# nekStab/nekStab_next

Hardware: AMD Instinct MI355X
Metric: Arnoldi-step GB/s (achieved HBM) + Ritz-value rel-err, N=1e8 m=128 (higher is better)
Workload: dtype f64

## Files before the change

### include/nekkrylov.h

```cpp
#ifndef NEKKRYLOV_H
#define NEKKRYLOV_H

#include <stddef.h>
#include <stdint.h>

#ifdef __cplusplus
extern "C" {
#endif

#define NKV_ABI_VERSION 3

#define NKV_TILE 4096
#define NKV_MAX_COLS 1024
#define NKV_ROT_MAX_OUT 256

#define NKV_OK 0
#define NKV_EINVAL 1
#define NKV_EHIP 2
#define NKV_ENAN 3
#define NKV_ESHAPE 4
#define NKV_ECALLBACK 5
#define NKV_EBREAKDOWN 6

#define NKV_TIME 0x1u
// ... 58 lines not shown
                void* stream);
int nkv_normalize_store(const nkv_layout* L, const double* f, const double* nrm2_dev, double* q_next,
                        double* beta_dev, unsigned flags, void* stream);
int nkv_mgs2_step(const nkv_layout* L, const double* w, const double* Q, int j, double* f, double* q_out,
                  double* hcol_dev, void* ws, unsigned flags, void* stream);
int nkv_axpy_dot(const nkv_layout* L, const double* w, double* f, const double* alpha_dev, const double* qa,
                 const double* qb, double* out_dev, void* ws, unsigned flags, void* stream);

int nkv_block_dot2(const nkv_layout* L, const double* w, const double* Q, int j, const double* x,
                   const double* y, double* h_dev, void* ws, unsigned flags, void* stream);
int nkv_dcgs2_coef(int m, const double* hq_dev, const double* hw_dev, const double* nrm_prev_dev, double* H_dev,
                   int64_t ldh, double* coef_dev, void* ws, void* stream);
int nkv_dcgs2_update(const nkv_layout* L, const double* w, const double* Q, int m, const double* coef_dev,
                     double* qj, const double* win, double* fout, double* nrm2_dev, void* ws, unsigned flags,
                     void* stream);

int nkv_mgs_icwy_solve(int j, double* G, int64_t ldg, const double* grow, const double* b, double* x,
                       void* stream);

int nkv_gkl_coef(int side, int m, const double* hq_dev, const double* hw_dev, double* M_dev, int64_t ldm,
                 double* A_self, double* r_self, const double* A_other, const double* r_other, int64_t lda,
                 double* coef_dev, void* ws, void* stream);

typedef int (*nkv_matvec_fn)(void* user, const double* x, double* y, void* stream);
typedef int (*nkv_allreduce_fn)(void* user, double* buf, int n, void* stream);
size_t nkv_arnoldi_scratch_doubles(int m);
int nkv_arnoldi_dcgs2(const nkv_layout* L, const double* w, double* Q, int mstart, int mend, double* H_dev,
                      int64_t ldh, double* f, double* scratch_dev, void* ws, nkv_matvec_fn matvec, void* mv_user,
                      nkv_allreduce_fn allreduce, void* ar_user, unsigned flags, void* stream);

// ... 22 lines not shown
int nkv_rotate_plan(const nkv_layout* L, int k, int ldv, int n_out, int* path, int* inst, int* wg_threads,
                    int* rows_per_tile);

#define NKV_STREAM_BLOCK_DOT 1
#define NKV_STREAM_BLOCK_UPDATE 2
#define NKV_STREAM_UPDATE_DOT 3
#define NKV_STREAM_BLOCK_DOT2 4
#define NKV_STREAM_DCGS2_UPDATE 5
#define NKV_STREAM_AXPY_DOT 6
#define NKV_STREAM_BLAS1 7
#define NKV_STREAM_OP_DIAG 8
#define NKV_STREAM_FINISH 9
#define NKV_STREAM_SPLIT 10
#define NKV_STREAM_LOOP_TILES 1
#define NKV_STREAM_LOOP_UNITS 2
typedef struct nkv_plan {
    int64_t kernel, pairs, nw, cpw, wg_threads, rows_per_tile, tiles, grid_x, grid_y, launches, band_tiles,
        last_grid_x, work_loop, units, fields_per_block, partial_slots, partial_cols;
} nkv_plan;
int nkv_stream_plan(const nkv_layout* L, int op, int j, unsigned flags, nkv_plan* plan);

int nkv_op_diag(const nkv_layout* L, const double* d, const double* x, double* y, double time_scale,
                void* stream);
int nkv_op_rot2(const nkv_layout* L, const double* c, const double* s, const double* d_rest,
                const double* x, double* y, int transpose, void* stream);
int nkv_op_cdiag(const nkv_layout* L, const double* cr, const double* ci, const double* x, double* y, int conj,
                 void* stream);

int nkv_wavemaker(const nkv_layout* L, const double* dRe, const double* dIm, const double* aRe, const double* aIm,
                  double* out, int ncomp, void* stream);
// ... 130 lines not shown
```

### nekstab_next_amd/_lib.py

```python
from __future__ import annotations

import ctypes
import os
from ctypes import CFUNCTYPE, POINTER, Structure, c_char_p, c_double, c_int, c_int32, c_int64, c_size_t, c_uint, c_uint64, c_void_p

import torch

_HERE = os.path.dirname(os.path.abspath(__file__))
LIB_PATH = os.path.join(_HERE, "libnekkrylov.so")

NKV_ABI_VERSION = 3
NKV_TILE = 4096
NKV_MAX_COLS = 1024
NKV_ROT_MAX_OUT = 256
NKV_GS_MAX_FIELDS = 64
NKV_ROT_PATH_FEW, NKV_ROT_PATH_WIDE, NKV_ROT_PATH_STREAM, NKV_ROT_PATH_CHUNKED = 1, 2, 3, 4
(NKV_STREAM_BLOCK_DOT, NKV_STREAM_BLOCK_UPDATE, NKV_STREAM_UPDATE_DOT, NKV_STREAM_BLOCK_DOT2, NKV_STREAM_DCGS2_UPDATE,
 NKV_STREAM_AXPY_DOT, NKV_STREAM_BLAS1, NKV_STREAM_OP_DIAG, NKV_STREAM_FINISH, NKV_STREAM_SPLIT) = range(1, 11)
NKV_STREAM_LOOP_TILES, NKV_STREAM_LOOP_UNITS = 1, 2
NKV_OK, NKV_EINVAL, NKV_EHIP, NKV_ENAN, NKV_ESHAPE, NKV_ECALLBACK, NKV_EBREAKDOWN = 0, 1, 2, 3, 4, 5, 6
NKV_TIME = 0x1
NKV_ACCUMULATE = 0x2
NKV_OVERWRITE = 0x4
NKV_NORM2 = 0x8
NKV_TIME_DOT = 0x10
NKV_X_IS_LAST = 0x20
NKV_MGS2 = 0x40
NKV_MGS_ICWY = 0x100
NKV_MGS_LAGGED = 0x200
NKV_CHECK_BREAKDOWN = 0x80
NKV_SFD_MONITOR = 0x400
NKV_TDF_STORE = 0x800
NKV_BF_IMAG = 0x1000
NKV_BF_PERTURBATION = 0x2000
# ... 51 lines not shown
    "nkv_copy": (c_int, [_L, _P, _P, c_uint, _P]),
    "nkv_scal": (c_int, [_L, _P, c_double, c_uint, _P]),
    "nkv_axpby": (c_int, [_L, _P, c_double, _P, c_double, c_uint, _P]),
    "nkv_sub3": (c_int, [_L, _P, _P, _P, c_uint, _P]),
    "nkv_axpy_dev": (c_int, [_L, _P, _P, c_double, _P, c_uint, _P]),
    "nkv_normalize_dev": (c_int, [_L, _P, _P, _P, c_uint, _P]),
    "nkv_dot": (c_int, [_L, _P, _P, _P, _P, _P, c_uint, _P]),
    "nkv_block_dot": (c_int, [_L, _P, _P, c_int, _P, _P, _P, c_uint, _P]),
    "nkv_block_update": (c_int, [_L, _P, _P, c_int, _P, _P, _P, _P, c_uint, _P]),
    "nkv_block_update_dot": (c_int, [_L, _P, _P, c_int, _P, _P, _P, _P, c_uint, _P]),
    "nkv_arnoldi_finish": (c_int, [_L, _P, _P, _P, c_int, _P, _P, _P, c_uint, _P]),
    "nkv_block_dot2": (c_int, [_L, _P, _P, c_int, _P, _P, _P, _P, c_uint, _P]),
    "nkv_dcgs2_coef": (c_int, [c_int, _P, _P, _P, _P, c_int64, _P, _P, _P]),
    "nkv_mgs_icwy_solve": (c_int, [c_int, _P, c_int64, _P, _P, _P, _P]),
    "nkv_dcgs2_update": (c_int, [_L, _P, _P, c_int, _P, _P, _P, _P, _P, _P, c_uint, _P]),
    "nkv_arnoldi_scratch_doubles": (c_size_t, [c_int]),
    "nkv_arnoldi_dcgs2": (c_int, [_L, _P, _P, c_int, c_int, _P, c_int64, _P, _P, _P, MATVEC_FN, _P, ALLREDUCE_FN, _P,
                                  c_uint, _P]),
    "nkv_update_hessenberg": (c_int, [_L, _P, _P, c_int, _P, _P, _P, _P, _P, ALLREDUCE_FN, _P, c_uint, _P]),
    "nkv_gmres_dcgs2": (c_int, [_L, _P, _P, c_int, c_double, c_double, _P, c_int64, _P, _P, _P, MATVEC_FN, _P,
                                ALLREDUCE_FN, _P, _P, _P, c_uint, _P]),
    "nkv_arnoldi_factorization": (c_int, [_L, _P, _P, c_int, c_int, _P, c_int64, _P, _P, _P, MATVEC_FN, _P,
                                          ALLREDUCE_FN, _P, c_uint, _P]),
    "nkv_combine": (c_int, [_L, _P, c_int, _P, _P, c_uint, _P]),
    "nkv_normalize_store": (c_int, [_L, _P, _P, _P, _P, c_uint, _P]),
    "nkv_mgs2_step": (c_int, [_L, _P, _P, c_int, _P, _P, _P, _P, c_uint, _P]),
    "nkv_axpy_dot": (c_int, [_L, _P, _P, _P, _P, _P, _P, _P, c_uint, _P]),
    "nkv_rotate": (c_int, [_L, _P, c_int, _P, c_int, _P]),
    "nkv_rotate_cols": (c_int, [_L, _P, c_int, _P, c_int, c_int, _P]),
    "nkv_rotate_plan": (c_int, [_L, c_int, c_int, c_int, POINTER(c_int), POINTER(c_int), POINTER(c_int),
# ... 107 lines not shown
```

### nekstab_next_amd/arnoldi.py

```python
from __future__ import annotations

import numpy as np
import torch

from . import _lib
from ._lib import NKV_NORM2, NKV_TIME, NKV_TIME_DOT, NKV_X_IS_LAST
from .operators import LinearOperator
from .vector import Basis, NekContext, NekVector


class HessenbergDev:

    def __init__(self, ctx: NekContext, k: int):
        self.ctx, self.k = ctx, k
        self.t = torch.zeros((k, k + 1), dtype=torch.float64, device=ctx.device)

    def col_ptr(self, c: int) -> int:
        return self.t[c].data_ptr()

    def download(self) -> np.ndarray:
        return np.asfortranarray(self.t.detach().cpu().numpy().T)

    def upload(self, H: np.ndarray) -> None:
        self.t.copy_(torch.as_tensor(np.ascontiguousarray(np.asarray(H, dtype=np.float64).T)).to(self.ctx.device))
# ... 68 lines not shown
                out = h[i + 1:i + 2] if not last else (h2[0:1] if p == 0 else nrm)
                ctx.call("nkv_axpy_dot", w, f.ptr, h[i:i + 1].data_ptr(), Q.col_ptr(i), qn, out.data_ptr(), ws, fl,
                         st)
                ctx.comm.allreduce_(out)
    else:
        raise ValueError(f"unknown orthogonalisation mode {mode!r}")
    if ctx.timer:
        ctx.timer.begin("finish")
    ctx.call("nkv_arnoldi_finish", f.ptr, nrm.data_ptr(), out_ptr, j, h1.data_ptr(), h2.data_ptr(),
             hcol_ptr, 0, st)
    if ctx.timer:
        ctx.timer.end("finish", 16.0 * ctx.layout.N)


def _dcgs2_step(ctx: NekContext, Q: Basis, Hd: HessenbergDev, j: int, f: NekVector, first: bool,
                nrm2: torch.Tensor | None = None) -> None:
    w, ws, st = ctx.w.data_ptr(), ctx.ws.data_ptr(), ctx.stream
    lay, tm = ctx.layout, ctx.timer
    tf = NKV_TIME if ctx.time_in_dot else 0
    m = j - 1
    h = ctx.hd[: 2 * j]
    hp, cp = h.data_ptr(), ctx.coef.data_ptr()
    u = Q.col_ptr(m)
    if tm:
        tm.begin("block_dot2")
    ctx.call("nkv_block_dot2", w, Q.ptr, j, u, f.ptr, hp, ws, tf | NKV_X_IS_LAST, st)
    if tm:
        tm.end("block_dot2", 8.0 * ((j - 1) * lay.N_w + 2 * lay.N_w + lay.n_v))
    ctx.comm.allreduce_(h)
    nprev = None if first else (nrm2.data_ptr() if nrm2 is not None else hp + 8 * m)
    ctx.call_nl("nkv_dcgs2_coef", m, hp, hp + 8 * j, nprev, Hd.t.data_ptr(), Hd.k + 1, cp, ws, st)
    if tm:
        tm.begin("dcgs2_update")
    ctx.call("nkv_dcgs2_update", w, Q.ptr, m, cp, u, f.ptr, Q.col_ptr(j), None if nrm2 is None else nrm2.data_ptr(),
             ws, NKV_TIME | (NKV_TIME_DOT if tf else 0), st)
    if tm:
        tm.end("dcgs2_update", 8.0 * (m * lay.N + 4 * lay.N) + (0.0 if nrm2 is None else 8.0 * lay.n_v))
    if nrm2 is not None:
        ctx.comm.allreduce_(nrm2)


def _dcgs2_close(ctx: NekContext, Q: Basis, Hd: HessenbergDev, m: int) -> None:
    w, ws, st = ctx.w.data_ptr(), ctx.ws.data_ptr(), ctx.stream
    lay, tm = ctx.layout, ctx.timer
    tf = NKV_TIME if ctx.time_in_dot else 0
    h, coef = ctx.hd[: m + 1], ctx.coef
    u = Q.col_ptr(m)
    if tm:
        tm.begin("block_dot")
    ctx.call("nkv_block_dot", w, Q.ptr, m + 1, u, h.data_ptr(), ws, tf, st)
    if tm:
        tm.end("block_dot", 8.0 * ((m + 1) * lay.N_w + lay.N_w + lay.n_v))
    ctx.comm.allreduce_(h)
    ctx.call_nl("nkv_dcgs2_coef", m, h.data_ptr(), None, h.data_ptr() + 8 * m, Hd.t.data_ptr(), Hd.k + 1,
                coef.data_ptr(), ws, st)
    if tm:
        tm.begin("block_update")
    ctx.call("nkv_block_update", w, Q.ptr, m, h.data_ptr(), u, None, ws, NKV_TIME, st)
    if tm:
        tm.end("block_update", 8.0 * (m * lay.N + 2 * lay.N))
    ctx.call("nkv_normalize_dev", u, coef[2 * m + 3:].data_ptr(), None, 0, st)


def _icwy_gram(ctx: NekContext, Q: Basis, mstart: int) -> torch.Tensor:
    ldg = ctx.max_cols + 1
    G = getattr(ctx, "_icwy_G", None)
    if G is None:
        G = ctx._icwy_G = torch.zeros((ldg, ldg), dtype=torch.float64, device=ctx.device)
    w, ws, st = ctx.w.data_ptr(), ctx.ws.data_ptr(), ctx.stream
    tf = NKV_TIME if ctx.time_in_dot else 0
    for i in range(1, mstart - 1):
        ctx.call("nkv_block_dot", w, Q.ptr, i, Q.col_ptr(i), G[i].data_ptr(), ws, tf, st)
        ctx.comm.allreduce_(G[i, :i])
    return G


# ... 183 lines not shown
        raise ValueError("basis too small")
    if f is None:
        f = ctx.vector()
    if mode == "dcgs2-native":
        if on_step is None:
            if mend > ctx.max_cols or mend + 1 > Hd.k + 1:
                raise ValueError(f"step {mend} exceeds max_cols {ctx.max_cols} / H size {Hd.k}")
            _dcgs2_native(ctx, op, Q, Hd, mstart, mend, f, transpose)
            return
        mode = "dcgs2"
    if mode == "dcgs2" and on_step is not None:
        if mend > ctx.max_cols or mend + 1 > Hd.k + 1:
            raise ValueError(f"step {mend} exceeds max_cols {ctx.max_cols} / H size {Hd.k}")
        for mstep in range(mstart, mend + 1):
            (op.rmatvec if transpose else op.matvec)(Q[mstep - 1], f)
            _dcgs2_step(ctx, Q, Hd, mstep, f, first=(mstep == mstart))
            if mstep > mstart:
                on_step(mstep - 1)
        _dcgs2_close(ctx, Q, Hd, mend)
        on_step(mend)
        return
    if mode == "mgs2-lagged-native":
        if on_step is None:
            if mend > ctx.max_cols or mend + 1 > Hd.k + 1:
                raise ValueError(f"step {mend} exceeds max_cols {ctx.max_cols} / H size {Hd.k}")
            _dcgs2_native(ctx, op, Q, Hd, mstart, mend, f, transpose, entry="nkv_arnoldi_factorization",
                          flags=_lib.NKV_MGS_LAGGED)
            return
        mode = "mgs2-lagged"
    if mode == "mgs2-lagged":
        if mend > ctx.max_cols or mend + 1 > Hd.k + 1:
# ... 17 lines not shown
            _icwy_step(ctx, Q, Hd, mstep, f, G)
            if on_step is not None:
                on_step(mstep)
        return
    if mode in ("cgs2-native", "mgs2-native") and on_step is None:
        if mend > ctx.max_cols or mend + 1 > Hd.k + 1:
            raise ValueError(f"step {mend} exceeds max_cols {ctx.max_cols} / H size {Hd.k}")
        _dcgs2_native(ctx, op, Q, Hd, mstart, mend, f, transpose, entry="nkv_arnoldi_factorization",
                      flags=_lib.NKV_MGS2 if mode == "mgs2-native" else 0)
        return
    if mode == "dcgs2" and on_step is None:
        if mend > ctx.max_cols or mend + 1 > Hd.k + 1:
            raise ValueError(f"step {mend} exceeds max_cols {ctx.max_cols} / H size {Hd.k}")
        for mstep in range(mstart, mend + 1):
            (op.rmatvec if transpose else op.matvec)(Q[mstep - 1], f)
            _dcgs2_step(ctx, Q, Hd, mstep, f, first=(mstep == mstart))
        _dcgs2_close(ctx, Q, Hd, mend)
        return
    if mode == "dcgs2":
        mode = "cgs2"
    for mstep in range(mstart, mend + 1):
        x = Q[mstep - 1]
        (op.rmatvec if transpose else op.matvec)(x, f)
        update_hessenberg_matrix(ctx, Q, mstep, f, Hd, mode)
        if on_step is not None:
            on_step(mstep)


class FactorizationGraph:

    def __init__(self, ctx: NekContext, op: LinearOperator, Q: Basis, Hd: HessenbergDev, f: NekVector,
# ... 26 lines not shown
```

### nekstab_next_amd/csrc/core.hip

```cpp
#include "nkv_internal.h"

namespace nkvi {

thread_local char g_err[512] = "";

int fail(int code, const char* fmt, ...) {
    va_list ap;
    va_start(ap, fmt);
    vsnprintf(g_err, sizeof(g_err), fmt, ap);
    va_end(ap);
    return code;
}

int device_cus() {
    static int cus[64] = {0};
    int dev = 0;
    if (hipGetDevice(&dev) != hipSuccess || dev < 0 || dev >= 64) return 256;
    if (!cus[dev]) {
        int n = 0;
        cus[dev] = (hipDeviceGetAttribute(&n, hipDeviceAttributeMultiprocessorCount, dev) == hipSuccess && n > 0)
                       ? n : 256;
    }
    return cus[dev];
}
// ... 172 lines not shown
            set_tile_grid(&p, L, large ? NKV_DC_PAIRS : NKV_PAIRS_SMALL, NKV_DC_G < kMaxBlocks ? NKV_DC_G : kMaxBlocks);
            if (!(flags & NKV_NORM2)) {
                set_bands(&p, NKV_DC_ROUNDS, true);
                break;
            }
            set_bands(&p, 0, true);
            const int64_t tpf = L->sv / p.rows_per_tile;
            if (!(tpf < p.grid_x && j >= 8)) {
                p.work_loop = NKV_STREAM_LOOP_UNITS;
                p.units = tpf + (p.tiles - tpf * L->n_wf);
            }
            p.partial_slots = p.grid_x;
            p.partial_cols = 1;
            break;
        }
        case NKV_STREAM_AXPY_DOT: {
            set_tile_grid(&p, L, NKV_PAIRS_SMALL, kMaxBlocks);
            set_bands(&p, NKV_AXD_ROUNDS, true);
            p.partial_slots = p.tiles > 0 ? p.grid_x : 0;
            p.partial_cols = 1;
            break;
        }
        case NKV_STREAM_BLAS1:
        case NKV_STREAM_FINISH:
        case NKV_STREAM_OP_DIAG: {
            p.pairs = kStreamUnr;
            p.wg_threads = kThreads;
            p.rows_per_tile = (int64_t)2 * kThreads * kStreamUnr;
            p.tiles = rows / p.rows_per_tile;
            p.grid_x = grid_for(op == NKV_STREAM_BLAS1 ? rows / 2 + 1 : rows / 2);
// ... 28 lines not shown
```

### nekstab_next_amd/csrc/drivers.hip

```cpp
#include "nkv_internal.h"

#include <vector>

extern "C" {

static size_t icwy_scratch_doubles(int m) { return (size_t)(4 * (m + 1) + 2) + (size_t)(m + 1) * (size_t)(m + 1); }
size_t nkv_arnoldi_scratch_doubles(int m) {
    const size_t base = (size_t)(2 * (m + 1) + 4 * m + 16), icwy = icwy_scratch_doubles(m);
    return base > icwy ? base : icwy;
}

static constexpr double kBreakdownTol = 1e-8;

static int check_breakdown(const double* H_dev, int64_t ldh, int c0, int c1, void* ws, void* stream) {
    if (c0 < 0) c0 = 0;
    if (c1 <= c0) return NKV_OK;
    hipStream_t st = S(stream);
    const size_t n = (size_t)ldh * (size_t)(c1 - c0);
    double* h = static_cast<double*>(malloc(n * sizeof(double)));
    if (!h) return fail(NKV_EINVAL, "breakdown check: host allocation of %zu doubles failed", n);
    int flag = 0;
    hipError_t e = hipMemcpyAsync(h, H_dev + (int64_t)c0 * ldh, n * sizeof(double), hipMemcpyDeviceToHost, st);
    if (e == hipSuccess) e = hipMemcpyAsync(&flag, nan_flag_of(ws), sizeof(int), hipMemcpyDeviceToHost, st);
    if (e == hipSuccess) e = hipStreamSynchronize(st);
// ... 34 lines not shown
    if (mend < mstart) return NKV_OK;
    if (ldh < mend + 1) return fail(NKV_EINVAL, "ldh=%lld < mend+1=%d", (long long)ldh, mend + 1);
    const unsigned tf = (flags & NKV_TIME_DOT) ? NKV_TIME : 0u;
    double* hd = scratch_dev;
    double* coef = scratch_dev + 2 * (mend + 1);
    auto col = [L, Q](int c) { return Q + (int64_t)c * L->ld; };
    for (int j = mstart; j <= mend; ++j) {
        const int m = j - 1;
        double* u = col(m);
        int rc = matvec(mv_user, u, f, stream);
        if (rc != 0) return fail(NKV_ECALLBACK, "matvec callback returned %d at step %d", rc, j);
        CHECK(nkv_block_dot2(L, w, Q, j, u, f, hd, ws, tf | NKV_X_IS_LAST, stream));
        if (allreduce && (rc = allreduce(ar_user, hd, 2 * j, stream)) != 0)
            return fail(NKV_ECALLBACK, "allreduce callback returned %d at step %d", rc, j);
        CHECK(nkv_dcgs2_coef(m, hd, hd + j, j == mstart ? nullptr : hd + m, H_dev, ldh, coef, ws, stream));
        CHECK(nkv_dcgs2_update(L, w, Q, m, coef, u, f, col(j), nullptr, ws, NKV_TIME, stream));
    }
    const int m = mend;
    double* u = col(m);
    CHECK(nkv_block_dot(L, w, Q, m + 1, u, hd, ws, tf, stream));
    if (allreduce) {
        const int rc = allreduce(ar_user, hd, m + 1, stream);
        if (rc != 0) return fail(NKV_ECALLBACK, "allreduce callback returned %d (closing step)", rc);
    }
    CHECK(nkv_dcgs2_coef(m, hd, nullptr, hd + m, H_dev, ldh, coef, ws, stream));
    CHECK(nkv_block_update(L, w, Q, m, hd, u, nullptr, ws, NKV_TIME, stream));
    CHECK(nkv_normalize_dev(L, u, coef + 2 * m + 3, nullptr, 0, stream));
    return (flags & NKV_CHECK_BREAKDOWN) ? check_breakdown(H_dev, ldh, mstart - 1, mend, ws, stream) : NKV_OK;
}

int nkv_gmres_dcgs2(const nkv_layout* L, const double* w, double* Q, int kmax, double beta, double tol2,
                    double* H_dev, int64_t ldh, double* f, double* scratch_dev, void* ws, nkv_matvec_fn matvec,
                    void* mv_user, nkv_allreduce_fn allreduce, void* ar_user, double* res_hist, int* k_out,
                    unsigned flags, void* stream) {
    CHECK(check_layout(L));
    CHECK(check_ptr(Q, "Q"));
    CHECK(check_ptr(f, "f"));
    CHECK(check_ptr(w, "w"));
    CHECK(check_ptr(ws, "ws"));
    if (!matvec) return fail(NKV_EINVAL, "matvec callback is NULL");
    if (!H_dev || !scratch_dev || !res_hist || !k_out) return fail(NKV_EINVAL, "H/scratch/res_hist/k_out is NULL");
    if (kmax < 1 || kmax + 1 > NKV_MAX_COLS) return fail(NKV_EINVAL, "kmax=%d outside 1..%d", kmax, NKV_MAX_COLS - 1);
// ... 325 lines not shown
```

### nekstab_next_amd/csrc/gram_schmidt.hip

```cpp
#include "nkv_internal.h"

namespace {

template <bool OVERWRITE, bool NORM, int kPairs>
__global__ __launch_bounds__(kThreads) void k_block_update(const double* __restrict__ Q, int64_t ld,
                                                           int j, const double* __restrict__ h,
                                                           double* __restrict__ f,
                                                           const double* __restrict__ w, int64_t sv,
                                                           int tiles_per_field, int tiles_w,
                                                           int tiles_total, int64_t time_off,
                                                           int do_time,
                                                           double* __restrict__ partials, int t_lo,
                                                           int acc_part) {
    constexpr int kTile = kThreads * kPairs * 2;
    __shared__ double lds4[4];
    if (do_time && blockIdx.x == 0 && threadIdx.x < 64) {
        double s = 0.0;
        for (int c = threadIdx.x; c < j; c += 64) s = fma(Q[time_off + (int64_t)c * ld], h[c], s);
        s = wave_sum(s);
        if (threadIdx.x == 0) f[time_off] = OVERWRITE ? s : f[time_off] - s;
    }
    double nrm = 0.0;
    for (int t = t_lo + blockIdx.x; t < tiles_total; t += gridDim.x) {
        const int64_t r0 = (int64_t)t * kTile + 2 * threadIdx.x;
        double2 acc[kPairs];
#pragma unroll
        for (int k = 0; k < kPairs; ++k) {
            if (OVERWRITE) acc[k] = make_double2(0.0, 0.0);
            else acc[k] = ld2(f + r0 + k * 2 * kThreads);
        }
        const double* qb = Q + r0;
        int c = 0;
        for (; c + 4 <= j; c += 4) {
            double2 q[4][kPairs];
#pragma unroll
// ... 6 lines not shown
#pragma unroll
                for (int k = 0; k < kPairs; ++k) {
                    acc[k].x = fma(hc, q[u][k].x, acc[k].x);
                    acc[k].y = fma(hc, q[u][k].y, acc[k].y);
                }
            }
        }
        for (; c < j; ++c) {
            const double hc = OVERWRITE ? h[c] : -h[c];
#pragma unroll
            for (int k = 0; k < kPairs; ++k) {
                const double2 q = ldq(qb + (int64_t)c * ld + k * 2 * kThreads);
                acc[k].x = fma(hc, q.x, acc[k].x);
                acc[k].y = fma(hc, q.y, acc[k].y);
            }
        }
#pragma unroll
        for (int k = 0; k < kPairs; ++k) st2(f + r0 + k * 2 * kThreads, acc[k]);
        if (NORM && t < tiles_w) {
            const int64_t wr = r0 - (int64_t)(t / tiles_per_field) * sv;
#pragma unroll
            for (int k = 0; k < kPairs; ++k) {
                const double2 wv = ld2(w + wr + k * 2 * kThreads);
                nrm = fma(wv.x * acc[k].x, acc[k].x, nrm);
                nrm = fma(wv.y * acc[k].y, acc[k].y, nrm);
            }
        }
    }
    if (NORM) {
        nrm = block_sum(nrm, lds4);
// ... 480 lines not shown
#pragma unroll
                for (int k = 0; k < kPairs; ++k) {
                    nrm = fma(wv[k].x * af[k].x, af[k].x, nrm);
                    nrm = fma(wv[k].y * af[k].y, af[k].y, nrm);
                }
            }
        } else {
            dcgs2_tile<kPairs>(Q, ld, m, a, x, rinv, yc, sc, qj, win, f,
                               (int64_t)(tiles_w + u - tiles_per_field) * kTile + 2 * threadIdx.x, af);
        }
    }
    nrm = block_sum(nrm, lds4);
    if (threadIdx.x == 0) partials[blockIdx.x] = nrm;
}

template <int P>
int launch_block_update_p(const nkv_layout* L, const nkv_plan& p, const double* w, const double* Q, int j,
                          const double* h_dev, double* f, double* part, unsigned flags, hipStream_t st) {
    const bool over = (flags & NKV_OVERWRITE) != 0;
    const bool norm = (flags & NKV_NORM2) != 0;
    const int tpf = (int)(L->sv / p.rows_per_tile);
    const int tiles_w = tpf * L->n_wf;
    const int tiles_total = (int)p.tiles;
    const int64_t T = rows_of(L);
    const int dt = (flags & NKV_TIME) ? 1 : 0;
    auto kern = over ? (norm ? k_block_update<true, true, P> : k_block_update<true, false, P>)
                     : (norm ? k_block_update<false, true, P> : k_block_update<false, false, P>);
    for (int64_t i = 0; i < p.launches; ++i) {
        const int lo = (int)(i * p.band_tiles);
        const int hi = lo + p.band_tiles < tiles_total ? (int)(lo + p.band_tiles) : tiles_total;
        const int64_t gb = i + 1 == p.launches ? p.last_grid_x : p.grid_x;
        hipLaunchKernelGGL(kern, dim3((unsigned)gb), dim3(kThreads), 0, st, Q, L->ld, j, h_dev, f, w, L->sv, tpf, tiles_w,
                           hi, T, lo == 0 ? dt : 0, part, lo, lo == 0 ? 0 : 1);
        NKV_LAUNCHED();
    }
    return NKV_OK;
}

__global__ __launch_bounds__(kThreads) void k_mgs_icwy_solve(int j, double* __restrict__ G, int64_t ldg,
                                                             const double* __restrict__ grow,
                                                             const double* b, double* x) {
    extern __shared__ double xs[];
    for (int i = threadIdx.x; i < j; i += kThreads) xs[i] = b[i];
    if (grow)
        for (int k = threadIdx.x; k < j - 1; k += kThreads) G[(int64_t)(j - 1) * ldg + k] = grow[k];
    for (int k = 0; k + 1 < j; ++k) {
        __syncthreads();
        const double xk = xs[k];
// ... 23 lines not shown
        CHECK(check_ptr(w, "w"));
        CHECK(check_ptr(ws, "ws"));
        if (!nrm2_dev) return fail(NKV_EINVAL, "nrm2_dev is NULL");
    }
    double* part = ws ? partials_of(ws) : nullptr;
    hipStream_t st = S(stream);
    const int g = (int)p.grid_x;
    const int64_t T = rows_of(L);
    if (p.pairs == NKV_PAIRS) CHECK(launch_block_update_p<NKV_PAIRS>(L, p, w, Q, j, h_dev, f, part, flags, st));
    else CHECK(launch_block_update_p<NKV_PAIRS_SMALL>(L, p, w, Q, j, h_dev, f, part, flags, st));
    if (norm) {
        const bool tdot = (flags & NKV_TIME_DOT) && L->rank0;
        CHECK(launch_reduce_cols(1, part, g, nrm2_dev, tdot ? f + T : nullptr, (int64_t)0, tdot ? f + T : nullptr, nullptr, 1 << 30, nan_flag_of(ws), st));
    }
    return NKV_OK;
}

int nkv_block_update_dot(const nkv_layout* L, const double* w, const double* Q, int j, const double* h_dev,
                         double* f, double* hout_dev, void* ws, unsigned flags, void* stream) {
    CHECK(check_layout(L));
    CHECK(check_ptr(w, "w"));
    CHECK(check_ptr(Q, "Q"));
    CHECK(check_ptr(f, "f"));
    CHECK(check_ptr(ws, "ws"));
    if (!h_dev || !hout_dev) return fail(NKV_EINVAL, "h_dev/hout_dev is NULL");
    nkv_plan p;
    CHECK(nkv_stream_plan(L, NKV_STREAM_UPDATE_DOT, j, flags, &p));
    const unsigned upd_flags = (flags & NKV_TIME) ? NKV_TIME : 0u;
    const unsigned dot_flags = (flags & NKV_TIME_DOT) ? NKV_TIME : 0u;
    if (p.kernel == NKV_STREAM_SPLIT) {
// ... 158 lines not shown
                      : (nrm2_dev ? k_dcgs2_update<NKV_PAIRS_SMALL, true> : k_dcgs2_update<NKV_PAIRS_SMALL, false>);
    for (int64_t i = 0; i < p.launches; ++i) {
        const int lo = (int)(i * p.band_tiles);
        const int hi = lo + p.band_tiles < tiles_total ? (int)(lo + p.band_tiles) : tiles_total;
        const int64_t gb = i + 1 == p.launches ? p.last_grid_x : p.grid_x;
        hipLaunchKernelGGL(kern, dim3((unsigned)gb), dim3(kThreads), 0, st, Q, L->ld, m, coef_dev, qj, win, fout, w, L->sv,
                           tpf, tiles_w, tiles_total, T, lo == 0 ? dt : 0, part, lo, hi);
        NKV_LAUNCHED();
    }
    if (!nrm2_dev) return NKV_OK;
    const bool tdot = (flags & NKV_TIME_DOT) && L->rank0;
    CHECK(launch_reduce_cols(1, part, g, nrm2_dev, tdot ? fout + T : nullptr, (int64_t)0, tdot ? fout + T : nullptr, nullptr, 1 << 30, nan_flag_of(ws), st));
    return NKV_OK;
}

int nkv_combine(const nkv_layout* L, const double* Q, int k, const double* y_dev, double* out, unsigned flags,
                void* stream) {
    return nkv_block_update(L, nullptr, Q, k, y_dev, out, nullptr, nullptr,
                            (flags & ~(unsigned)NKV_NORM2) | NKV_OVERWRITE, stream);
}

}
```

### nekstab_next_amd/csrc/nkv_internal.h

```cpp
#pragma once

#include <hip/hip_runtime.h>

#include <cmath>
#include <cstdarg>
#include <cstdio>
#include <cstdlib>
#include <cstring>

#include "nekkrylov.h"

#ifndef NKV_PAIRS
#define NKV_PAIRS 8
#endif
#ifndef NKV_PAIRS_SMALL
#define NKV_PAIRS_SMALL 4
#endif
#ifndef NKV_SMALL_TILES
#define NKV_SMALL_TILES 2048
#endif
#ifndef NKV_COLU
#define NKV_COLU 4
#endif
#ifndef NKV_NT
// ... 37 lines not shown
#endif
#ifndef NKV_AXD_ROUNDS
#define NKV_AXD_ROUNDS 0
#endif
#ifndef NKV_UPD_SMALL_J
#define NKV_UPD_SMALL_J 2
#endif
#ifndef NKV_FUSE_SMALL_J
#define NKV_FUSE_SMALL_J 12
#endif
static_assert(NKV_FUSE_SMALL_J >= 0 && NKV_FUSE_SMALL_J <= 16,
              "the 4-wave fused pass instantiates at most 16 columns (NKV_FUSE(4, 4))");
#ifndef NKV_FUSE_ROUNDS
#define NKV_FUSE_ROUNDS 0
#endif
#ifndef NKV_DC_ROUNDS
#define NKV_DC_ROUNDS 2
#endif
#ifndef NKV_STREAM_ROUNDS
#define NKV_STREAM_ROUNDS 2
#endif
#ifndef NKV_D2_MAXB
#define NKV_D2_MAXB 256
#endif
#ifndef NKV_D2_SMALL_B
#define NKV_D2_SMALL_B 512
#endif
#ifndef NKV_DOT_SMALL_B
#define NKV_DOT_SMALL_B 512
#endif
// ... 296 lines not shown
```

### nekstab_next_amd/vector.py

```python
from __future__ import annotations

import ctypes

import numpy as np
import torch

from . import _lib
from ._lib import NKV_OVERWRITE, NKV_TIME
from .comm import Comm
from .layout import NekLayout


def _ptr(t: torch.Tensor) -> int:
    return t.data_ptr()


class NekContext:

    def __init__(self, layout: NekLayout, weights=None, comm: Comm | None = None, max_cols: int = 256,
                 device: torch.device | int | None = None, time_in_dot: bool = False):
        if not 1 <= max_cols < _lib.NKV_MAX_COLS:
            raise ValueError(f"max_cols={max_cols} outside 1..{_lib.NKV_MAX_COLS - 1}")
        _lib.require_gpu()
        self.comm = comm if comm is not None else Comm()
# ... 258 lines not shown
                _lib.NKV_ROT_PATH_CHUNKED: "chunked"}


def rotate_plan(layout, k: int, n_out: int, ldv: int | None = None) -> tuple[str, int, int, int]:
    L = layout.c_struct() if isinstance(layout, NekLayout) else layout
    out = [ctypes.c_int(0) for _ in range(4)]
    rc = _lib.load().nkv_rotate_plan(ctypes.byref(L), int(k), int(k if ldv is None else ldv), int(n_out),
                                     *[ctypes.byref(o) for o in out])
    _lib.check(rc, "nkv_rotate_plan")
    return ROTATE_PATHS[out[0].value], out[1].value, out[2].value, out[3].value


STREAM_OPS = {"block_dot": _lib.NKV_STREAM_BLOCK_DOT, "block_update": _lib.NKV_STREAM_BLOCK_UPDATE,
              "update_dot": _lib.NKV_STREAM_UPDATE_DOT, "block_dot2": _lib.NKV_STREAM_BLOCK_DOT2,
              "dcgs2_update": _lib.NKV_STREAM_DCGS2_UPDATE, "axpy_dot": _lib.NKV_STREAM_AXPY_DOT,
              "blas1": _lib.NKV_STREAM_BLAS1, "op_diag": _lib.NKV_STREAM_OP_DIAG, "finish": _lib.NKV_STREAM_FINISH}
_STREAM_KERNELS = {**{v: k for k, v in STREAM_OPS.items()}, _lib.NKV_STREAM_SPLIT: "split"}
_STREAM_LOOPS = {0: None, _lib.NKV_STREAM_LOOP_TILES: "tiles", _lib.NKV_STREAM_LOOP_UNITS: "units"}


class StreamPlan(dict):

    __getattr__ = dict.__getitem__


def stream_plan(layout, op: str, j: int = 1, flags: int = 0) -> StreamPlan:
    L = layout.c_struct() if isinstance(layout, NekLayout) else layout
    p = _lib.nkv_plan()
    _lib.check(_lib.load().nkv_stream_plan(ctypes.byref(L), STREAM_OPS[op], int(j), int(flags), ctypes.byref(p)),
               "nkv_stream_plan")
    out = StreamPlan((name, int(getattr(p, name))) for name, _ in p._fields_)
# ... 12 lines not shown
```

Before: 6764.

## Fuse closing block-dot into final DCGS2 update and scale in block update

The last Arnoldi step now uses a new fused kernel that performs the DCGS2 update and computes the closing dot products against all basis columns while the tiles are still in registers, so the separate block_dot pass over Q is no longer needed. The closing normalize is folded into the block update through a scaled variant that multiplies by the inverse norm before storing. Together these drop one full read of the basis and one vector pass per Arnoldi cycle. The cost is a more complex kernel with LDS cross-wave reductions and a per-tile barrier, plus many template instantiations. Large m or very large row counts fall back to the split path.

Measured after the change: 6753. About the same (-0.2%).

```diff
diff --git a/include/nekkrylov.h b/include/nekkrylov.h
--- a/include/nekkrylov.h
+++ b/include/nekkrylov.h
@@ -96,6 +96,11 @@
 int nkv_dcgs2_update(const nkv_layout* L, const double* w, const double* Q, int m, const double* coef_dev,
                      double* qj, const double* win, double* fout, double* nrm2_dev, void* ws, unsigned flags,
                      void* stream);
+int nkv_dcgs2_update_dot(const nkv_layout* L, const double* w, const double* Q, int m, const double* coef_dev,
+                         double* qj, const double* win, double* fout, double* hout_dev, void* ws, unsigned flags,
+                         void* stream);
+int nkv_block_update_scaled(const nkv_layout* L, const double* Q, int j, const double* h_dev, double* f,
+                            const double* nrm2_dev, void* stream);
 
 int nkv_mgs_icwy_solve(int j, double* G, int64_t ldg, const double* grow, const double* b, double* x,
                        void* stream);
@@ -148,6 +153,7 @@
 #define NKV_STREAM_SPLIT 10
 #define NKV_STREAM_LOOP_TILES 1
 #define NKV_STREAM_LOOP_UNITS 2
+#define NKV_PLAN_DCGS2_UPDATE_DOT 12
 typedef struct nkv_plan {
     int64_t kernel, pairs, nw, cpw, wg_threads, rows_per_tile, tiles, grid_x, grid_y, launches, band_tiles,
         last_grid_x, work_loop, units, fields_per_block, partial_slots, partial_cols;
diff --git a/nekstab_next_amd/_lib.py b/nekstab_next_amd/_lib.py
--- a/nekstab_next_amd/_lib.py
+++ b/nekstab_next_amd/_lib.py
@@ -18,6 +18,7 @@
 (NKV_STREAM_BLOCK_DOT, NKV_STREAM_BLOCK_UPDATE, NKV_STREAM_UPDATE_DOT, NKV_STREAM_BLOCK_DOT2, NKV_STREAM_DCGS2_UPDATE,
  NKV_STREAM_AXPY_DOT, NKV_STREAM_BLAS1, NKV_STREAM_OP_DIAG, NKV_STREAM_FINISH, NKV_STREAM_SPLIT) = range(1, 11)
 NKV_STREAM_LOOP_TILES, NKV_STREAM_LOOP_UNITS = 1, 2
+NKV_PLAN_DCGS2_UPDATE_DOT = 12
 NKV_OK, NKV_EINVAL, NKV_EHIP, NKV_ENAN, NKV_ESHAPE, NKV_ECALLBACK, NKV_EBREAKDOWN = 0, 1, 2, 3, 4, 5, 6
 NKV_TIME = 0x1
 NKV_ACCUMULATE = 0x2
@@ -99,6 +100,8 @@
     "nkv_dcgs2_coef": (c_int, [c_int, _P, _P, _P, _P, c_int64, _P, _P, _P]),
     "nkv_mgs_icwy_solve": (c_int, [c_int, _P, c_int64, _P, _P, _P, _P]),
     "nkv_dcgs2_update": (c_int, [_L, _P, _P, c_int, _P, _P, _P, _P, _P, _P, c_uint, _P]),
+    "nkv_dcgs2_update_dot": (c_int, [_L, _P, _P, c_int, _P, _P, _P, _P, _P, _P, c_uint, _P]),
+    "nkv_block_update_scaled": (c_int, [_L, _P, c_int, _P, _P, _P, _P]),
     "nkv_arnoldi_scratch_doubles": (c_size_t, [c_int]),
     "nkv_arnoldi_dcgs2": (c_int, [_L, _P, _P, c_int, c_int, _P, c_int64, _P, _P, _P, MATVEC_FN, _P, ALLREDUCE_FN, _P,
                                   c_uint, _P]),
diff --git a/nekstab_next_amd/arnoldi.py b/nekstab_next_amd/arnoldi.py
--- a/nekstab_next_amd/arnoldi.py
+++ b/nekstab_next_amd/arnoldi.py
@@ -106,7 +106,9 @@
 
 
 def _dcgs2_step(ctx: NekContext, Q: Basis, Hd: HessenbergDev, j: int, f: NekVector, first: bool,
-                nrm2: torch.Tensor | None = None) -> None:
+                nrm2: torch.Tensor | None = None, last: bool = False) -> None:
+    if last and nrm2 is not None:
+        raise ValueError("last=True: the closing dots supply the norm; nrm2 must be None")
     w, ws, st = ctx.w.data_ptr(), ctx.ws.data_ptr(), ctx.stream
     lay, tm = ctx.layout, ctx.timer
     tf = NKV_TIME if ctx.time_in_dot else 0
@@ -124,6 +126,12 @@
     ctx.call_nl("nkv_dcgs2_coef", m, hp, hp + 8 * j, nprev, Hd.t.data_ptr(), Hd.k + 1, cp, ws, st)
     if tm:
         tm.begin("dcgs2_update")
+    if last:
+        ctx.call("nkv_dcgs2_update_dot", w, Q.ptr, m, cp, u, f.ptr, Q.col_ptr(j), hp, ws,
+                 NKV_TIME | (NKV_TIME_DOT if tf else 0), st)
+        if tm:
+            tm.end("dcgs2_update", 8.0 * (m * lay.N + 4 * lay.N + lay.n_v))
+        return
     ctx.call("nkv_dcgs2_update", w, Q.ptr, m, cp, u, f.ptr, Q.col_ptr(j), None if nrm2 is None else nrm2.data_ptr(),
              ws, NKV_TIME | (NKV_TIME_DOT if tf else 0), st)
     if tm:
@@ -133,25 +141,18 @@
 
 
 def _dcgs2_close(ctx: NekContext, Q: Basis, Hd: HessenbergDev, m: int) -> None:
-    w, ws, st = ctx.w.data_ptr(), ctx.ws.data_ptr(), ctx.stream
+    st = ctx.stream
     lay, tm = ctx.layout, ctx.timer
-    tf = NKV_TIME if ctx.time_in_dot else 0
     h, coef = ctx.hd[: m + 1], ctx.coef
     u = Q.col_ptr(m)
-    if tm:
-        tm.begin("block_dot")
-    ctx.call("nkv_block_dot", w, Q.ptr, m + 1, u, h.data_ptr(), ws, tf, st)
-    if tm:
-        tm.end("block_dot", 8.0 * ((m + 1) * lay.N_w + lay.N_w + lay.n_v))
     ctx.comm.allreduce_(h)
     ctx.call_nl("nkv_dcgs2_coef", m, h.data_ptr(), None, h.data_ptr() + 8 * m, Hd.t.data_ptr(), Hd.k + 1,
-                coef.data_ptr(), ws, st)
+                coef.data_ptr(), ctx.ws.data_ptr(), st)
     if tm:
         tm.begin("block_update")
-    ctx.call("nkv_block_update", w, Q.ptr, m, h.data_ptr(), u, None, ws, NKV_TIME, st)
+    ctx.call("nkv_block_update_scaled", Q.ptr, m, h.data_ptr(), u, coef[2 * m + 3:].data_ptr(), st)
     if tm:
         tm.end("block_update", 8.0 * (m * lay.N + 2 * lay.N))
-    ctx.call("nkv_normalize_dev", u, coef[2 * m + 3:].data_ptr(), None, 0, st)
 
 
 def _icwy_gram(ctx: NekContext, Q: Basis, mstart: int) -> torch.Tensor:
@@ -365,7 +366,7 @@
             raise ValueError(f"step {mend} exceeds max_cols {ctx.max_cols} / H size {Hd.k}")
         for mstep in range(mstart, mend + 1):
             (op.rmatvec if transpose else op.matvec)(Q[mstep - 1], f)
-            _dcgs2_step(ctx, Q, Hd, mstep, f, first=(mstep == mstart))
+            _dcgs2_step(ctx, Q, Hd, mstep, f, first=(mstep == mstart), last=(mstep == mend))
             if mstep > mstart:
                 on_step(mstep - 1)
         _dcgs2_close(ctx, Q, Hd, mend)
@@ -413,7 +414,7 @@
             raise ValueError(f"step {mend} exceeds max_cols {ctx.max_cols} / H size {Hd.k}")
         for mstep in range(mstart, mend + 1):
             (op.rmatvec if transpose else op.matvec)(Q[mstep - 1], f)
-            _dcgs2_step(ctx, Q, Hd, mstep, f, first=(mstep == mstart))
+            _dcgs2_step(ctx, Q, Hd, mstep, f, first=(mstep == mstart), last=(mstep == mend))
         _dcgs2_close(ctx, Q, Hd, mend)
         return
     if mode == "dcgs2":
diff --git a/nekstab_next_amd/csrc/core.hip b/nekstab_next_amd/csrc/core.hip
--- a/nekstab_next_amd/csrc/core.hip
+++ b/nekstab_next_amd/csrc/core.hip
@@ -210,6 +210,29 @@
             p.partial_cols = 1;
             break;
         }
+        case NKV_PLAN_DCGS2_UPDATE_DOT: {
+            if (j < 0 || j + 2 > NKV_MAX_COLS) return fail(NKV_EINVAL, "m=%d outside 0..%d", j, NKV_MAX_COLS - 2);
+            if (j > NKV_DCF_MAX_M || rows >= (int64_t)1 << 29) {
+                p.kernel = NKV_STREAM_SPLIT;
+                break;
+            }
+            p.nw = j <= NKV_FUSE_SMALL_J ? 4 : 8;
+            p.cpw = j > 0 ? (j + p.nw - 1) / p.nw : 1;
+            p.pairs = 1;
+            p.wg_threads = p.nw * 64;
+            p.rows_per_tile = kFuseRows;
+            p.tiles = rows / kFuseRows;
+            p.grid_x = p.tiles < NKV_DCF_G ? p.tiles : NKV_DCF_G;
+            if (p.grid_x < 1) p.grid_x = 1;
+            p.grid_y = 1;
+            p.work_loop = NKV_STREAM_LOOP_TILES;
+            p.units = p.tiles;
+            p.fields_per_block = 1;
+            set_bands(&p, 0, true);
+            p.partial_slots = p.grid_x;
+            p.partial_cols = j + 2;
+            break;
+        }
         case NKV_STREAM_AXPY_DOT: {
             set_tile_grid(&p, L, NKV_PAIRS_SMALL, kMaxBlocks);
             set_bands(&p, NKV_AXD_ROUNDS, true);
diff --git a/nekstab_next_amd/csrc/drivers.hip b/nekstab_next_amd/csrc/drivers.hip
--- a/nekstab_next_amd/csrc/drivers.hip
+++ b/nekstab_next_amd/csrc/drivers.hip
@@ -72,18 +72,21 @@
         if (allreduce && (rc = allreduce(ar_user, hd, 2 * j, stream)) != 0)
             return fail(NKV_ECALLBACK, "allreduce callback returned %d at step %d", rc, j);
         CHECK(nkv_dcgs2_coef(m, hd, hd + j, j == mstart ? nullptr : hd + m, H_dev, ldh, coef, ws, stream));
-        CHECK(nkv_dcgs2_update(L, w, Q, m, coef, u, f, col(j), nullptr, ws, NKV_TIME, stream));
+        if (j < mend) {
+            CHECK(nkv_dcgs2_update(L, w, Q, m, coef, u, f, col(j), nullptr, ws, NKV_TIME, stream));
+        } else {
+            CHECK(nkv_dcgs2_update_dot(L, w, Q, m, coef, u, f, col(j), hd, ws, NKV_TIME | (tf ? NKV_TIME_DOT : 0u),
+                                       stream));
+        }
     }
     const int m = mend;
     double* u = col(m);
-    CHECK(nkv_block_dot(L, w, Q, m + 1, u, hd, ws, tf, stream));
     if (allreduce) {
         const int rc = allreduce(ar_user, hd, m + 1, stream);
         if (rc != 0) return fail(NKV_ECALLBACK, "allreduce callback returned %d (closing step)", rc);
     }
     CHECK(nkv_dcgs2_coef(m, hd, nullptr, hd + m, H_dev, ldh, coef, ws, stream));
-    CHECK(nkv_block_update(L, w, Q, m, hd, u, nullptr, ws, NKV_TIME, stream));
-    CHECK(nkv_normalize_dev(L, u, coef + 2 * m + 3, nullptr, 0, stream));
+    CHECK(nkv_block_update_scaled(L, Q, m, hd, u, coef + 2 * m + 3, stream));
     return (flags & NKV_CHECK_BREAKDOWN) ? check_breakdown(H_dev, ldh, mstart - 1, mend, ws, stream) : NKV_OK;
 }
 
diff --git a/nekstab_next_amd/csrc/gram_schmidt.hip b/nekstab_next_amd/csrc/gram_schmidt.hip
--- a/nekstab_next_amd/csrc/gram_schmidt.hip
+++ b/nekstab_next_amd/csrc/gram_schmidt.hip
@@ -2,7 +2,7 @@
 
 namespace {
 
-template <bool OVERWRITE, bool NORM, int kPairs>
+template <bool OVERWRITE, bool NORM, int kPairs, bool SCALE = false>
 __global__ __launch_bounds__(kThreads) void k_block_update(const double* __restrict__ Q, int64_t ld,
                                                            int j, const double* __restrict__ h,
                                                            double* __restrict__ f,
@@ -11,14 +11,20 @@
                                                            int tiles_total, int64_t time_off,
                                                            int do_time,
                                                            double* __restrict__ partials, int t_lo,
-                                                           int acc_part) {
+                                                           int acc_part,
+                                                           const double* __restrict__ scale2 = nullptr) {
     constexpr int kTile = kThreads * kPairs * 2;
     __shared__ double lds4[4];
+    double inv = 1.0;
+    if constexpr (SCALE) inv = 1.0 / sqrt(scale2[0]);
     if (do_time && blockIdx.x == 0 && threadIdx.x < 64) {
         double s = 0.0;
         for (int c = threadIdx.x; c < j; c += 64) s = fma(Q[time_off + (int64_t)c * ld], h[c], s);
         s = wave_sum(s);
-        if (threadIdx.x == 0) f[time_off] = OVERWRITE ? s : f[time_off] - s;
+        if (threadIdx.x == 0) {
+            const double ft = OVERWRITE ? s : f[time_off] - s;
+            f[time_off] = SCALE ? ft * inv : ft;
+        }
     }
     double nrm = 0.0;
     for (int t = t_lo + blockIdx.x; t < tiles_total; t += gridDim.x) {
@@ -55,6 +61,10 @@
                 acc[k].x = fma(hc, q.x, acc[k].x);
                 acc[k].y = fma(hc, q.y, acc[k].y);
             }
+        }
+        if constexpr (SCALE) {
+#pragma unroll
+            for (int k = 0; k < kPairs; ++k) acc[k] = make_double2(acc[k].x * inv, acc[k].y * inv);
         }
 #pragma unroll
         for (int k = 0; k < kPairs; ++k) st2(f + r0 + k * 2 * kThreads, acc[k]);
@@ -565,9 +575,123 @@
     if (threadIdx.x == 0) partials[blockIdx.x] = nrm;
 }
 
+template <int NW, int CPW>
+__global__ __launch_bounds__(NW * 64) void k_dcgs2_update_dot(const double* __restrict__ Q, int64_t ld, int m,
+                                                               const double* __restrict__ coef,
+                                                               double* __restrict__ qj,
+                                                               const double* __restrict__ win,
+                                                               double* __restrict__ f,
+                                                               const double* __restrict__ w, int64_t sv,
+                                                               int64_t tiles_per_field, int64_t tiles_w,
+                                                               int64_t tiles_total, int64_t time_off,
+                                                               int do_time, double* __restrict__ partials,
+                                                               int B) {
+    static_assert(NW >= 2, "wave 0 owns qbar, wave 1 owns f");
+    __shared__ double2 part[2][NW][2][64];
+    const int wv = __builtin_amdgcn_readfirstlane(threadIdx.x >> 6);
+    const int lane = threadIdx.x & 63;
+    const double* x = coef;
+    const double* a = coef + 2 * m + 5;
+    const double rinv = coef[2 * m + 1], yc = coef[2 * m + 2], sc = coef[2 * m + 4];
+    const double wsc = sc * rinv;
+    if (do_time && blockIdx.x == 0 && wv == 0) {
+        double s1 = 0.0, s2 = 0.0;
+        for (int c = lane; c < m; c += 64) {
+            const double qt = Q[time_off + (int64_t)c * ld];
+            s1 = fma(qt, a[c], s1);
+            s2 = fma(qt, x[c], s2);
+        }
+        s1 = wave_sum(s1);
+        s2 = wave_sum(s2);
+        if (lane == 0) {
+            const double qb = (qj[time_off] * sc - s1) * rinv;
+            qj[time_off] = qb;
+            f[time_off] = win[time_off] * wsc - s2 - qb * yc;
+        }
+    }
+    __shared__ double2 cf[NW * CPW];
+    for (int c = threadIdx.x; c < NW * CPW; c += NW * 64) cf[c] = c < m ? make_double2(-a[c], -x[c]) : make_double2(0.0, 0.0);
+    __syncthreads();
+    const double* qcol[CPW];
+    double acc[CPW];
+#pragma unroll
+    for (int i = 0; i < CPW; ++i) {
+        const int c = wv + NW * i;
+        qcol[i] = Q + (int64_t)(c < m ? c : 0) * ld;
+        acc[i] = 0.0;
+    }
+    double accq = 0.0, accf = 0.0;
+    int buf = 0;
+    for (int64_t t = blockIdx.x; t < tiles_total; t += gridDim.x, buf ^= 1) {
+        const uint32_t r = (uint32_t)(t * kFuseRows) + 2u * lane;
+        const uint32_t rb = r * 8u;
+        double2 q[CPW];
+#pragma unroll
+        for (int i = 0; i < CPW - 1; ++i) q[i] = ldq(at_b(qcol[i], rb));
+        q[CPW - 1] = (wv + NW * (CPW - 1) < m) ? ldq(at_b(qcol[CPW - 1], rb)) : make_double2(0.0, 0.0);
+        double2 sa = make_double2(0.0, 0.0), sx = make_double2(0.0, 0.0);
+        if (wv == 0) {
+            const double2 uv = ld2(at_b(qj, rb));
+            sa = make_double2(uv.x * sc, uv.y * sc);
+        } else if (wv == 1) {
+            const double2 fv = ld2(at_b(win, rb));
+            sx = make_double2(fv.x * wsc, fv.y * wsc);
+        }
+        const bool weighted = t < tiles_w;
+        const double2 ww = weighted ? ld2(at_b(w, (r - (uint32_t)((t / tiles_per_field) * sv)) * 8u)) : make_double2(0.0, 0.0);
+#pragma unroll
+        for (int i = 0; i < CPW; ++i) {
+            const double2 cc = cf[wv + NW * i];
+            sa.x = fma(cc.x, q[i].x, sa.x);
+            sa.y = fma(cc.x, q[i].y, sa.y);
+            sx.x = fma(cc.y, q[i].x, sx.x);
+            sx.y = fma(cc.y, q[i].y, sx.y);
+        }
+        part[buf][wv][0][lane] = sa;
+        part[buf][wv][1][lane] = sx;
+        __syncthreads();
+        double2 ta = part[buf][0][0][lane], tx = part[buf][0][1][lane];
+#pragma unroll
+        for (int k = 1; k < NW; ++k) {
+            const double2 pa = part[buf][k][0][lane], px = part[buf][k][1][lane];
+            ta.x += pa.x;
+            ta.y += pa.y;
+            tx.x += px.x;
+            tx.y += px.y;
+        }
+        const double2 qbv = make_double2(ta.x * rinv, ta.y * rinv);
+        const double2 fo = make_double2(fma(-yc, qbv.x, tx.x), fma(-yc, qbv.y, tx.y));
+        if (wv == 0) st2s(const_cast<double*>(at_b(qj, rb)), qbv);
+        if (wv == 1) st2s(const_cast<double*>(at_b(f, rb)), fo);
+        if (weighted) {
+            const double wa = ww.x * fo.x, wb = ww.y * fo.y;
+#pragma unroll
+            for (int i = 0; i < CPW; ++i) acc[i] = fma(q[i].y, wb, fma(q[i].x, wa, acc[i]));
+            if (wv == 0) {
+                accq = fma(qbv.y, wb, fma(qbv.x, wa, accq));
+                accf = fma(fo.y, wb, fma(fo.x, wa, accf));
+            }
+        }
+    }
+#pragma unroll
+    for (int i = 0; i < CPW; ++i) {
+        const int c = wv + NW * i;
+        const double v = wave_sum(acc[i]);
+        if (lane == 0 && c < m) partials[(int64_t)c * B + blockIdx.x] = v;
+    }
+    if (wv == 0) {
+        const double vq = wave_sum(accq), vf = wave_sum(accf);
+        if (lane == 0) {
+            partials[(int64_t)m * B + blockIdx.x] = vq;
+            partials[(int64_t)(m + 1) * B + blockIdx.x] = vf;
+        }
+    }
+}
+
 template <int P>
 int launch_block_update_p(const nkv_layout* L, const nkv_plan& p, const double* w, const double* Q, int j,
-                          const double* h_dev, double* f, double* part, unsigned flags, hipStream_t st) {
+                          const double* h_dev, double* f, double* part, unsigned flags, hipStream_t st,
+                          const double* scale2 = nullptr) {
     const bool over = (flags & NKV_OVERWRITE) != 0;
     const bool norm = (flags & NKV_NORM2) != 0;
     const int tpf = (int)(L->sv / p.rows_per_tile);
@@ -577,12 +701,13 @@
     const int dt = (flags & NKV_TIME) ? 1 : 0;
     auto kern = over ? (norm ? k_block_update<true, true, P> : k_block_update<true, false, P>)
                      : (norm ? k_block_update<false, true, P> : k_block_update<false, false, P>);
+    if (scale2) kern = k_block_update<false, false, P, true>;
     for (int64_t i = 0; i < p.launches; ++i) {
         const int lo = (int)(i * p.band_tiles);
         const int hi = lo + p.band_tiles < tiles_total ? (int)(lo + p.band_tiles) : tiles_total;
         const int64_t gb = i + 1 == p.launches ? p.last_grid_x : p.grid_x;
         hipLaunchKernelGGL(kern, dim3((unsigned)gb), dim3(kThreads), 0, st, Q, L->ld, j, h_dev, f, w, L->sv, tpf, tiles_w,
-                           hi, T, lo == 0 ? dt : 0, part, lo, lo == 0 ? 0 : 1);
+                           hi, T, lo == 0 ? dt : 0, part, lo, lo == 0 ? 0 : 1, scale2);
         NKV_LAUNCHED();
     }
     return NKV_OK;
@@ -636,6 +761,19 @@
         CHECK(launch_reduce_cols(1, part, g, nrm2_dev, tdot ? f + T : nullptr, (int64_t)0, tdot ? f + T : nullptr, nullptr, 1 << 30, nan_flag_of(ws), st));
     }
     return NKV_OK;
+}
+
+int nkv_block_update_scaled(const nkv_layout* L, const double* Q, int j, const double* h_dev, double* f,
+                            const double* nrm2_dev, void* stream) {
+    CHECK(check_layout(L));
+    CHECK(check_ptr(Q, "Q"));
+    CHECK(check_ptr(f, "f"));
+    if (!h_dev || !nrm2_dev) return fail(NKV_EINVAL, "h_dev/nrm2_dev is NULL");
+    nkv_plan p;
+    CHECK(nkv_stream_plan(L, NKV_STREAM_BLOCK_UPDATE, j, 0u, &p));
+    if (p.pairs == NKV_PAIRS)
+        return launch_block_update_p<NKV_PAIRS>(L, p, nullptr, Q, j, h_dev, f, nullptr, NKV_TIME, S(stream), nrm2_dev);
+    return launch_block_update_p<NKV_PAIRS_SMALL>(L, p, nullptr, Q, j, h_dev, f, nullptr, NKV_TIME, S(stream), nrm2_dev);
 }
 
 int nkv_block_update_dot(const nkv_layout* L, const double* w, const double* Q, int j, const double* h_dev,
@@ -824,6 +962,72 @@
     return NKV_OK;
 }
 
+int nkv_dcgs2_update_dot(const nkv_layout* L, const double* w, const double* Q, int m, const double* coef_dev,
+                         double* qj, const double* win, double* fout, double* hout_dev, void* ws, unsigned flags,
+                         void* stream) {
+    CHECK(check_layout(L));
+    CHECK(check_ptr(w, "w"));
+    CHECK(check_ptr(Q, "Q"));
+    CHECK(check_ptr(qj, "qj"));
+    CHECK(check_ptr(win, "win"));
+    CHECK(check_ptr(fout, "fout"));
+    CHECK(check_ptr(ws, "ws"));
+    nkv_plan p;
+    CHECK(nkv_stream_plan(L, NKV_PLAN_DCGS2_UPDATE_DOT, m, flags, &p));
+    if (!coef_dev || !hout_dev) return fail(NKV_EINVAL, "coef/hout_dev is NULL");
+    if (qj != Q + (int64_t)m * L->ld || fout != Q + (int64_t)(m + 1) * L->ld)
+        return fail(NKV_EINVAL, "dcgs2_update_dot: qj / fout are not columns m / m+1 of Q");
+    const unsigned dot_flags = (flags & NKV_TIME_DOT) ? NKV_TIME : 0u;
+    if (p.kernel == NKV_STREAM_SPLIT) {
+        CHECK(nkv_dcgs2_update(L, w, Q, m, coef_dev, qj, win, fout, nullptr, ws, flags & NKV_TIME, stream));
+        return launch_block_dot(L, w, Q, L->ld, m + 2, fout, hout_dev, ws, dot_flags, S(stream));
+    }
+    const int64_t tpf = L->sv / kFuseRows;
+    const int64_t tiles_w = tpf * L->n_wf;
+    const int B = (int)p.partial_slots;
+    const int64_t T = rows_of(L);
+    const int dt = (flags & NKV_TIME) ? 1 : 0;
+    double* part = partials_of(ws);
+    hipStream_t st = S(stream);
+#define NKV_DCF(NW, CPW)                                                                                           \
+    hipLaunchKernelGGL((k_dcgs2_update_dot<NW, CPW>), dim3((unsigned)p.grid_x), dim3(NW * 64), 0, st, Q, L->ld, m, \
+                       coef_dev, qj, win, fout, w, L->sv, tpf, tiles_w, p.tiles, T, dt, part, B)
+    const int cpw = (int)p.cpw;
+    if (p.nw == 4) {
+        switch (cpw) {
+            case 1: NKV_DCF(4, 1); break;
+            case 2: NKV_DCF(4, 2); break;
+            case 3: NKV_DCF(4, 3); break;
+            default: NKV_DCF(4, 4); break;
+        }
+    } else {
+        switch (cpw) {
+            case 1: NKV_DCF(8, 1); break;
+            case 2: NKV_DCF(8, 2); break;
+            case 3: NKV_DCF(8, 3); break;
+            case 4: NKV_DCF(8, 4); break;
+            case 5: NKV_DCF(8, 5); break;
+            case 6: NKV_DCF(8, 6); break;
+            case 7: NKV_DCF(8, 7); break;
+            case 8: NKV_DCF(8, 8); break;
+            case 9: NKV_DCF(8, 9); break;
+            case 10: NKV_DCF(8, 10); break;
+            case 11: NKV_DCF(8, 11); break;
+            case 12: NKV_DCF(8, 12); break;
+            case 13: NKV_DCF(8, 13); break;
+            case 14: NKV_DCF(8, 14); break;
+            case 15: NKV_DCF(8, 15); break;
+            default: NKV_DCF(8, 16); break;
+        }
+    }
+#undef NKV_DCF
+    NKV_LAUNCHED();
+    const bool tdot = dot_flags && L->rank0;
+    CHECK(launch_reduce_cols(m + 2, part, B, hout_dev, tdot ? Q + T : nullptr, L->ld, tdot ? fout + T : nullptr, nullptr,
+                             1 << 30, nan_flag_of(ws), st));
+    return NKV_OK;
+}
+
 int nkv_combine(const nkv_layout* L, const double* Q, int k, const double* y_dev, double* out, unsigned flags,
                 void* stream) {
     return nkv_block_update(L, nullptr, Q, k, y_dev, out, nullptr, nullptr,
diff --git a/nekstab_next_amd/csrc/nkv_internal.h b/nekstab_next_amd/csrc/nkv_internal.h
--- a/nekstab_next_amd/csrc/nkv_internal.h
+++ b/nekstab_next_amd/csrc/nkv_internal.h
@@ -75,6 +75,14 @@
 #ifndef NKV_FUSE_ROUNDS
 #define NKV_FUSE_ROUNDS 0
 #endif
+#ifndef NKV_DCF_G
+#define NKV_DCF_G 1024
+#endif
+#ifndef NKV_DCF_MAX_M
+#define NKV_DCF_MAX_M 128
+#endif
+static_assert(NKV_DCF_MAX_M >= 0 && NKV_DCF_MAX_M <= 128 && NKV_DCF_G <= NKV_MAXB,
+              "k_dcgs2_update_dot: 8 waves x 16 columns at the most; kMaxBlocks partial slots per column");
 #ifndef NKV_DC_ROUNDS
 #define NKV_DC_ROUNDS 2
 #endif
diff --git a/nekstab_next_amd/vector.py b/nekstab_next_amd/vector.py
--- a/nekstab_next_amd/vector.py
+++ b/nekstab_next_amd/vector.py
@@ -296,7 +296,8 @@
 STREAM_OPS = {"block_dot": _lib.NKV_STREAM_BLOCK_DOT, "block_update": _lib.NKV_STREAM_BLOCK_UPDATE,
               "update_dot": _lib.NKV_STREAM_UPDATE_DOT, "block_dot2": _lib.NKV_STREAM_BLOCK_DOT2,
               "dcgs2_update": _lib.NKV_STREAM_DCGS2_UPDATE, "axpy_dot": _lib.NKV_STREAM_AXPY_DOT,
-              "blas1": _lib.NKV_STREAM_BLAS1, "op_diag": _lib.NKV_STREAM_OP_DIAG, "finish": _lib.NKV_STREAM_FINISH}
+              "blas1": _lib.NKV_STREAM_BLAS1, "op_diag": _lib.NKV_STREAM_OP_DIAG, "finish": _lib.NKV_STREAM_FINISH,
+              "dcgs2_update_dot": _lib.NKV_PLAN_DCGS2_UPDATE_DOT}
 _STREAM_KERNELS = {**{v: k for k, v in STREAM_OPS.items()}, _lib.NKV_STREAM_SPLIT: "split"}
 _STREAM_LOOPS = {0: None, _lib.NKV_STREAM_LOOP_TILES: "tiles", _lib.NKV_STREAM_LOOP_UNITS: "units"}
 
```
